# xxlong0/ESTDepth

Measured on AMD Instinct MI355X. Metric: depth frames/sec (seq_len=5, 480x640, D=64), higher is better.
Workload: dtype f32; 1 GPU; cfg2: seq_len=5, 480x640, ndepths=64, ResNet-50, Joint mode steady state (carried memory, EST on); launch=hipGraph replay, pipeline=False, graph_memory=zero-copy, conv3d_arith=f32, conv2d_arith=f32, conv3d_algo_32to32=wino3, full=False, parallelism=1 sequence per GPU

## Files before the change

estdepth_amd/csrc/conv3d_wino3.hip:

```cpp
#include <hip/hip_runtime.h>
#include <stdint.h>
#include <stdlib.h>
#include <type_traits>

#include "estd_hip.h"
#include "estd_common.h"

#ifndef ESTD_W3BD
#define ESTD_W3BD 4
#endif
#ifndef ESTD_W3_SCHED
#define ESTD_W3_SCHED 1
#endif
#ifndef ESTD_W3_WRING
#define ESTD_W3_WRING 0
#endif
#ifndef ESTD_W3_RBQ
#define ESTD_W3_RBQ 5
#endif
#ifndef ESTD_W3_TANH_HALVES
#define ESTD_W3_TANH_HALVES 1
#endif
#ifndef ESTD_W3_PFQ
#define ESTD_W3_PFQ 4
#endif
#ifndef ESTD_W3_PFQ_RB
#define ESTD_W3_PFQ_RB 8
#endif
#ifndef ESTD_W3PRIO
#define ESTD_W3PRIO 0
#endif
#ifndef ESTD_W3PK
#define ESTD_W3PK 0
#endif
#ifndef ESTD_W3_SCHED_VALU
#define ESTD_W3_SCHED_VALU 8
#endif
#ifndef ESTD_W3ABL
#define ESTD_W3ABL 0
#endif

namespace {

typedef float f32x4 __attribute__((ext_vector_type(4)));
typedef float f32x2 __attribute__((ext_vector_type(2)));
typedef unsigned int u32x4 __attribute__((__vector_size__(16)));

constexpr int TH = 8, TW = 16;
constexpr int IN_H = TH + 2, IN_W = TW + 2;
constexpr int SL_VOX = IN_H * IN_W;
constexpr int SL_CHUNKS = SL_VOX * 8;
constexpr int LINE_BYTES = IN_W * 128 + 16;
constexpr int ROW_BYTES = 4 * LINE_BYTES;
constexpr int SLICE_BYTES = LINE_BYTES;
constexpr int SLICES_BYTES = IN_H * ROW_BYTES;
constexpr int NTHREADS = 512, SIT = 3;
constexpr int RED_BYTES = 512;
constexpr int SS_BYTES = 3 * 32 * 4;
constexpr int VTAB_BYTES = SIT * NTHREADS * 4;
constexpr int XCH_BYTES = 8 * 4 * 64 * 16;
constexpr int NTAPS = 64, TAP_BYTES = 4096;
constexpr int DUMMY_BYTES = 96 * 16 + 2 * LINE_BYTES;
constexpr int XSL_BYTES = 4 * SL_VOX * 4;
constexpr int XW_BYTES = 2 * 4 * 2 * 64 * 16;
constexpr int LDS_BASE_BYTES = SLICES_BYTES + RED_BYTES + SS_BYTES + VTAB_BYTES + XCH_BYTES + DUMMY_BYTES;
#ifndef ESTD_W3_WLDS
#define ESTD_W3_WLDS 1
#endif
#ifndef ESTD_W3_WLQ0_PLAIN
#define ESTD_W3_WLQ0_PLAIN 4
#endif
constexpr int WL_N = 3;
constexpr int WL_BYTES = 2 * WL_N * 4096;
constexpr int LDS_BYTES_EXTRA = LDS_BASE_BYTES + XSL_BYTES + XW_BYTES, LDS_BYTES_PLAIN = LDS_BASE_BYTES + (ESTD_W3_WLDS ? WL_BYTES : 0);
static_assert(LDS_BYTES_EXTRA <= 160 * 1024 && LDS_BYTES_PLAIN <= 160 * 1024, "LDS budget");
constexpr unsigned OOB_OFFSET = 0xFFFFFF00u;

__device__ __forceinline__ float4 as_float4(u32x4 v)
{
    float4 f;
    __builtin_memcpy(&f, &v, 16);
    return f;
}
__device__ __forceinline__ __amdgpu_buffer_rsrc_t make_rsrc(const float* base, size_t elems)
{
    return __builtin_amdgcn_make_buffer_rsrc(const_cast<float*>(base), 0, (int)(elems * 4), 0x00020000);
}
template <int CTRL>
__device__ __forceinline__ double dpp_add_f64(double v)
{
    const unsigned long long b = __builtin_bit_cast(unsigned long long, v);
    const unsigned lo = (unsigned)__builtin_amdgcn_update_dpp(0, (int)(unsigned)b, CTRL, 0xf, 0xf, false);
    const unsigned hi = (unsigned)__builtin_amdgcn_update_dpp(0, (int)(unsigned)(b >> 32), CTRL, 0xf, 0xf, false);
    return v + __builtin_bit_cast(double, ((unsigned long long)hi << 32) | lo);
}
__device__ __forceinline__ double row16_sum_f64(double v)
{
    v = dpp_add_f64<0xB1>(v);
    v = dpp_add_f64<0x4E>(v);
    v = dpp_add_f64<0x124>(v);
    v = dpp_add_f64<0x128>(v);
    return v;
}
__device__ __forceinline__ void lds_barrier() { asm volatile("s_waitcnt lgkmcnt(0)\n\ts_barrier" ::: "memory"); }
__device__ __forceinline__ int lds_colkey_off(int col, int c) { return col * 128 + ((c ^ ((col >> 1) & 7)) << 4); }
__device__ __forceinline__ float tanh_fast(float x)
{
    const float t = __builtin_amdgcn_exp2f(x * 2.8853900817779268f);
    return 1.0f - 2.0f * __builtin_amdgcn_rcpf(t + 1.0f);
}
__device__ __forceinline__ float act_apply(float v, int act)
{
    if (act == ESTD_ACT_RELU) return v > 0.0f ? v : 0.0f;
    if (act == ESTD_ACT_TANH) return tanh_fast(v);
    return v;
}
__device__ __forceinline__ float4 f4_sub(float4 a, float4 b) { return make_float4(a.x - b.x, a.y - b.y, a.z - b.z, a.w - b.w); }
__device__ __forceinline__ float4 f4_add(float4 a, float4 b) { return make_float4(a.x + b.x, a.y + b.y, a.z + b.z, a.w + b.w); }

#ifndef ESTD_W3DEFER
#define ESTD_W3DEFER 1
#endif
template <int RBK, bool STATS, bool EXTRA>
__global__ __launch_bounds__(NTHREADS, 1) void conv3d_wino3_kernel(const estd_conv3d_desc p, int tiles_w, int tiles_h, int dpairs, int total_tiles)
{
    constexpr bool RB_ACC = RBK == 1 || RBK == 3, RB_RES = RBK == 2 || RBK == 3;
    constexpr bool DEFER = ESTD_W3DEFER != 0;
    extern __shared__ __attribute__((aligned(16))) char smem[];
    const int tid = threadIdx.x;
    const int lane = tid & 63;
    const int wave = __builtin_amdgcn_readfirstlane(tid >> 6);
    const int rq = wave & 1;
    const int nh = (wave >> 1) & 1;
    const int shh = wave >> 2;
    const int g = lane >> 4;
    const int i = lane & 15;
    const int rpl = (i >= 4 && i < 12) ? 1 : 0;
    const int cb = i < 4 ? i : i < 12 ? i - 4 : i - 8;
    const int D = p.D, H = p.H, W = p.W;
    const int HW = H * W;
    const size_t vol = (size_t)D * HW;

    int u, u_end;
    {
        const int G = gridDim.x, bid = blockIdx.x;
        const int r = ((G & 7) == 0) ? (bid & 7) * (G >> 3) + (bid >> 3) : bid;
        u = (int)((long long)total_tiles * r / G);
        u_end = (int)((long long)total_tiles * (r + 1) / G);
    }
    if (u >= u_end) return;

    float* lds_ss = reinterpret_cast<float*>(smem + SLICES_BYTES + RED_BYTES);
    if (tid < 64) lds_ss[tid] = tid < 32 ? p.scale[tid & 31] : p.shift[tid & 31];
    if (tid >= 64 && tid < 96) lds_ss[tid] = ((tid - 64) < p.act_split ? p.act_a : p.act_b) == ESTD_ACT_RELU ? 0.0f : ESTD_NO_FLOOR;
    const bool any_tanh = p.act_a == ESTD_ACT_TANH || p.act_b == ESTD_ACT_TANH;
    const bool tanh_halves = ESTD_W3_TANH_HALVES && any_tanh && (p.act_split & 15) == 0;
    const int wave_act = __builtin_amdgcn_readfirstlane(16 * nh < p.act_split ? p.act_a : p.act_b);
    unsigned* lds_vt = reinterpret_cast<unsigned*>(smem + SLICES_BYTES + RED_BYTES + SS_BYTES);
    float4* lds_xch = reinterpret_cast<float4*>(smem + SLICES_BYTES + RED_BYTES + SS_BYTES + VTAB_BYTES);
    const __amdgpu_buffer_rsrc_t rs_null = __builtin_amdgcn_make_buffer_rsrc(const_cast<float*>(p.w_wino2), 0, 0, 0x00020000);
    float* lds_x = reinterpret_cast<float*>(smem + SLICES_BYTES + RED_BYTES + SS_BYTES + VTAB_BYTES + XCH_BYTES + DUMMY_BYTES);
    char* lds_wx = smem + SLICES_BYTES + RED_BYTES + SS_BYTES + VTAB_BYTES + XCH_BYTES + DUMMY_BYTES + XSL_BYTES;
    if (EXTRA) {
        for (int e = tid; e < XW_BYTES / 16; e += NTHREADS) reinterpret_cast<float4*>(lds_wx)[e] = reinterpret_cast<const float4*>(p.w_extra)[e];
    }
    constexpr bool WL = ESTD_W3_WLDS != 0 && !EXTRA;
    constexpr int WL_Q0 = RBK == 0 ? ESTD_W3_WLQ0_PLAIN : 4;
    char* lds_wl = smem + LDS_BASE_BYTES;
    if (WL) {
        for (int e = tid; e < WL_BYTES / 16; e += NTHREADS) {
            const int blk = e >> 8, q_ = WL_Q0 + blk % WL_N, sh_ = 2 * (blk / WL_N) + (q_ & 1);
            const int src = ((((q_ >> 3) * 4 + sh_) * 2 + ((q_ >> 2) & 1)) * 2 + ((q_ >> 1) & 1));
            reinterpret_cast<float4*>(lds_wl)[e] = reinterpret_cast<const float4*>(p.w_wino2)[src * 256 + (e & 255)];
        }
    }
    const int xbase = ((4 * rq + 2 * rpl) * IN_W + 2 * cb) * 4 + g * (SL_VOX * 4);

    const __amdgpu_buffer_rsrc_t rs_w = make_rsrc(p.w_wino2, (size_t)NTAPS * 1024);
    const int wlane = lane * 16 + nh * 2048;
    int cbase[4][2][2];
#pragma unroll
    for (int j = 0; j < 4; ++j)
#pragma unroll
        for (int cc = 0; cc < 2; ++cc)
#pragma unroll
            for (int hh = 0; hh < 2; ++hh) cbase[j][cc][hh] = (4 * rq + 2 * rpl) * ROW_BYTES + lds_colkey_off(2 * cb + j, g + 4 * cc) + 8 * (hh ^ (g & 1));

    constexpr int BD = ESTD_W3BD;
    static_assert(32 % BD == 0, "the weight ring runs on across tiles");
    if (ESTD_W3PRIO == 1 && shh != 0) __builtin_amdgcn_s_setprio(1);
    while (u < u_end) {
        const int col = u / dpairs;
        int dp = u - col * dpairs;
        const int twi = col % tiles_w, c2 = col / tiles_w;
        const int thi = c2 % tiles_h, n = c2 / tiles_h;
        const int tw0 = twi * TW, th0 = thi * TH;
        const int seg_end = min(u_end, (col + 1) * dpairs);

        const __amdgpu_buffer_rsrc_t rs_in = make_rsrc(p.in_main + (size_t)n * vol * p.in_stride, vol * p.in_stride);
        __amdgpu_buffer_rsrc_t rs_res = rs_in, rs_res2 = rs_in;
        const __amdgpu_buffer_rsrc_t rs_out = make_rsrc(p.out_main + (size_t)n * vol * p.out_stride, vol * p.out_stride);
        rs_res = (RB_RES && p.residual) ? make_rsrc(p.residual + (size_t)n * vol * p.out_stride, vol * p.out_stride) : rs_null;
        rs_res2 = (RB_RES && p.residual2) ? make_rsrc(p.residual2 + (size_t)n * vol * p.out_stride, vol * p.out_stride) : rs_null;
        const __amdgpu_buffer_rsrc_t rs_ex = EXTRA ? make_rsrc(p.in_extra + (size_t)n * vol, vol) : rs_null;
        unsigned xoff = OOB_OFFSET;
        if (EXTRA && tid < SL_VOX) {
            const int zy = tid / IN_W, zx = tid % IN_W;
            const int gy = th0 - 1 + zy, gx = tw0 - 1 + zx;
            if ((unsigned)gy < (unsigned)H && (unsigned)gx < (unsigned)W) xoff = (unsigned)(gy * W + gx) * 4u;
        }
        auto load_x = [&](int pd) {
            return (unsigned)pd < (unsigned)D ? __builtin_bit_cast(float, __builtin_amdgcn_raw_buffer_load_b32(rs_ex, xoff, pd * HW * 4, 0)) : 0.0f;
        };
        const int in_slice_bytes = HW * p.in_stride * 4;
        const int out_plane_bytes = HW * p.out_stride * 4;

#pragma unroll
        for (int it = 0; it < SIT; ++it) {
            const int e = tid + it * NTHREADS;
            const int vs = e >> 3, c = e & 7;
            const int zy = vs / IN_W, zx = vs % IN_W;
            const int gy = th0 - 1 + zy, gx = tw0 - 1 + zx;
            const bool ok = e < SL_CHUNKS && (unsigned)gy < (unsigned)H && (unsigned)gx < (unsigned)W;
            lds_vt[it * NTHREADS + tid] = ok ? (unsigned)((gy * W + gx) * p.in_stride + c * 4) * 4u : OOB_OFFSET;
        }
        auto chunk_voff = [&](int it) {
            const int l = __builtin_amdgcn_mbcnt_hi(~0u, __builtin_amdgcn_mbcnt_lo(~0u, 0u));
            return lds_vt[it * NTHREADS + wave * 64 + l];
        };
        int loffk[SIT];
#pragma unroll
        for (int it = 0; it < SIT; ++it) {
            const int vs = (tid >> 3) + it * (NTHREADS / 8);
            loffk[it] = (vs / IN_W) * ROW_BYTES + lds_colkey_off(vs % IN_W, tid & 7);
        }
        const bool last_ok = tid + (SIT - 1) * NTHREADS < SL_CHUNKS;
        int loffw[SIT];
#pragma unroll
        for (int it = 0; it < SIT; ++it) loffw[it] = (it < SIT - 1 || last_ok) ? loffk[it] : (SLICES_BYTES + RED_BYTES + SS_BYTES + VTAB_BYTES + XCH_BYTES + (tid - 416) * 16);
        auto load_plane = [&](int pd, float4 (&dst)[SIT]) {
            const bool pv = (unsigned)pd < (unsigned)D;
#pragma unroll
            for (int it = 0; it < SIT; ++it)
                dst[it] = pv ? as_float4(__builtin_amdgcn_raw_buffer_load_b128(rs_in, chunk_voff(it), pd * in_slice_bytes, 0)) : make_float4(0.f, 0.f, 0.f, 0.f);
        };
        unsigned eoff[2][2];
#pragma unroll
        for (int m = 0; m < 2; ++m)
#pragma unroll
            for (int c = 0; c < 2; ++c) {
                const int y = th0 + 4 * rq + 2 * rpl + m, x = tw0 + 2 * cb + c;
                eoff[m][c] = (y < H && x < W) ? (unsigned)((y * W + x) * p.out_stride + 16 * nh + 4 * g) * 4u : OOB_OFFSET;
            }
        auto bn_act = [&](const f32x4& a, int chb, float4& v) {
            const float4 sc4 = *reinterpret_cast<const float4*>(lds_ss + chb), sh4 = *reinterpret_cast<const float4*>(lds_ss + 32 + chb);
            if (!any_tanh) {
                const float4 lo = *reinterpret_cast<const float4*>(lds_ss + 64 + chb);
                v.x = fmaxf(a[0] * sc4.x + sh4.x, lo.x);
                v.y = fmaxf(a[1] * sc4.y + sh4.y, lo.y);
                v.z = fmaxf(a[2] * sc4.z + sh4.z, lo.z);
                v.w = fmaxf(a[3] * sc4.w + sh4.w, lo.w);
                return;
            }
            if (tanh_halves) {
                const float u0 = a[0] * sc4.x + sh4.x, u1 = a[1] * sc4.y + sh4.y, u2 = a[2] * sc4.z + sh4.z, u3 = a[3] * sc4.w + sh4.w;
                if (wave_act == ESTD_ACT_TANH) { v.x = tanh_fast(u0); v.y = tanh_fast(u1); v.z = tanh_fast(u2); v.w = tanh_fast(u3); }
                else if (wave_act == ESTD_ACT_RELU) { v.x = fmaxf(u0, 0.f); v.y = fmaxf(u1, 0.f); v.z = fmaxf(u2, 0.f); v.w = fmaxf(u3, 0.f); }
                else { v.x = u0; v.y = u1; v.z = u2; v.w = u3; }
                return;
            }
            v.x = act_apply(a[0] * sc4.x + sh4.x, chb + 0 < p.act_split ? p.act_a : p.act_b);
            v.y = act_apply(a[1] * sc4.y + sh4.y, chb + 1 < p.act_split ? p.act_a : p.act_b);
            v.z = act_apply(a[2] * sc4.z + sh4.z, chb + 2 < p.act_split ? p.act_a : p.act_b);
            v.w = act_apply(a[3] * sc4.w + sh4.w, chb + 3 < p.act_split ? p.act_a : p.act_b);
        };
        struct EpiLoads { float4 r1[2], r2[2], ro[2]; };
        auto epi_issue = [&](int m, int so, const __amdgpu_buffer_rsrc_t& q1, const __amdgpu_buffer_rsrc_t& q2, const __amdgpu_buffer_rsrc_t& qo, EpiLoads& L) {
#pragma unroll
            for (int c = 0; c < 2; ++c) {
                if (RB_RES) L.r1[c] = as_float4(__builtin_amdgcn_raw_buffer_load_b128(q1, eoff[m][c], so, 0));
                if (RB_RES) L.r2[c] = as_float4(__builtin_amdgcn_raw_buffer_load_b128(q2, eoff[m][c], so, 0));
                if (RB_ACC) L.ro[c] = as_float4(__builtin_amdgcn_raw_buffer_load_b128(qo, eoff[m][c], so, 0));
            }
        };
        auto epi_finish = [&](const f32x4 (&a)[2], int m, int so, const __amdgpu_buffer_rsrc_t& qo, const EpiLoads& L) {
#pragma unroll
            for (int c = 0; c < 2; ++c) {
                float4 v;
                bn_act(a[c], 16 * nh + 4 * g, v);
                if (RB_RES) {
                    v = f4_add(f4_add(v, L.r1[c]), L.r2[c]);
                    v = make_float4(v.x * p.out_scale, v.y * p.out_scale, v.z * p.out_scale, v.w * p.out_scale);
                }
                if (RB_ACC) v = f4_add(v, L.ro[c]);
                u32x4 bits;
                __builtin_memcpy(&bits, &v, 16);
                if (!(ESTD_W3ABL & 1)) __builtin_amdgcn_raw_buffer_store_b128(bits, qo, eoff[m][c], so, 0);
            }
        };
        auto epi_plane = [&](const f32x4 (&a)[2][2], int dd) {
            const int so = dd * out_plane_bytes;
            EpiLoads L0, L1;
            epi_issue(0, so, rs_res, rs_res2, rs_out, L0);
            epi_issue(1, so, rs_res, rs_res2, rs_out, L1);
            epi_finish(a[0], 0, so, rs_out, L0);
            epi_finish(a[1], 1, so, rs_out, L1);
        };
        f32x4 py[2][2];
        int pso = 0;
        bool have_prev = false;
#pragma unroll
        for (int m = 0; m < 2; ++m)
#pragma unroll
            for (int c = 0; c < 2; ++c) py[m][c] = (f32x4){0.f, 0.f, 0.f, 0.f};

        float4 xa[SIT], xb[SIT], xc[SIT], xd[SIT];
        {
            const int d0 = 2 * dp;
            load_plane(d0 - 1, xa);
            load_plane(d0, xb);
            load_plane(d0 + 1, xc);
            load_plane(d0 + 2, xd);
        }
        float ea = 0.f, eb = 0.f, ec = 0.f, ed = 0.f;
        if (EXTRA) {
            const int d0 = 2 * dp;
            ea = load_x(d0 - 1); eb = load_x(d0); ec = load_x(d0 + 1); ed = load_x(d0 + 2);
        }
        char* xw_ptr = tid < SL_VOX ? reinterpret_cast<char*>(lds_x) + tid * 4 : smem + SLICES_BYTES + RED_BYTES + SS_BYTES + VTAB_BYTES + XCH_BYTES + (tid & 63) * 4;
        auto write_x_slice = [&](int sl) {
            if (EXTRA) *reinterpret_cast<float*>(xw_ptr + sl * (SL_VOX * 4)) = sl == 0 ? ea - ec : sl == 1 ? eb + ec : sl == 2 ? ec - eb : eb - ed;
        };
        auto write_slice = [&](int sl) {
#pragma unroll
            for (int it = 0; it < SIT; ++it) {
                if ((it < SIT - 1 || last_ok) && !(ESTD_W3ABL & 2)) {
                    const float4 v = sl == 0 ? f4_sub(xa[it], xc[it]) : sl == 1 ? f4_add(xb[it], xc[it])
                                   : sl == 2 ? f4_sub(xc[it], xb[it]) : f4_sub(xb[it], xd[it]);
                    *reinterpret_cast<float4*>(smem + loffk[it] + sl * SLICE_BYTES) = v;
                }
            }
        };
        auto shift_planes = [&]() {
#pragma unroll
            for (int it = 0; it < SIT; ++it) { xa[it] = xc[it]; xb[it] = xd[it]; }
            if (EXTRA) { ea = ec; eb = ed; }
        };
        bool first = true;
        int stats_parity = 0;
        float4 bq[BD][2];
        bool w_primed = false;

        for (; u < seg_end; ++u, ++dp) {
            const int d0 = 2 * dp;
            if (first) {
                lds_barrier();
#pragma unroll
                for (int sl = 0; sl < 4; ++sl) write_slice(sl);
#pragma unroll
                for (int sl = 0; sl < 4; ++sl) write_x_slice(sl);
                shift_planes();
                lds_barrier();
                first = false;
            }
            const bool has_next = (u + 1 < seg_end);
            const int nd = d0 + 3;
            const __amdgpu_buffer_rsrc_t rs_pf0 = (has_next && nd < D) ? rs_in : rs_null, rs_pf1 = (has_next && nd + 1 < D) ? rs_in : rs_null;
            const __amdgpu_buffer_rsrc_t rs_px0 = (EXTRA && has_next && nd < D) ? rs_ex : rs_null, rs_px1 = (EXTRA && has_next && nd + 1 < D) ? rs_ex : rs_null;

            f32x4 P[2][2][2];
            const __amdgpu_buffer_rsrc_t rp_out = have_prev ? rs_out : rs_null, rp_res = have_prev ? rs_res : rs_null, rp_res2 = have_prev ? rs_res2 : rs_null;

            auto tap_loop = [&](auto shh_c) {
                constexpr int SHH = decltype(shh_c)::value;
                constexpr int NQ = 32;
                constexpr int RA0 = SHH == 0 ? 0 : 2, RSH = SHH == 0 ? 2 : 1, RA1 = SHH == 0 ? 1 : 3;
                f32x4 m[2][4];
                f32x2 RA[4], RBs[4];
                f32x2 T[4];

                auto load_w = [&](int q, float4 (&b)[2]) {
                    const int sd = q >> 3, cc = (q >> 2) & 1, hh = (q >> 1) & 1, sh = 2 * SHH + (q & 1);
#pragma unroll
                    for (int sp = 0; sp < 2; ++sp) {
                        if (WL && q >= WL_Q0 && q < WL_Q0 + WL_N) b[sp] = *reinterpret_cast<const float4*>(lds_wl + (SHH * WL_N + q - WL_Q0) * 4096 + sp * 1024 + wlane);
                        else b[sp] = as_float4(__builtin_amdgcn_raw_buffer_load_b128(rs_w, wlane, ((((sd * 4 + sh) * 2 + cc) * 2 + hh) * TAP_BYTES) + sp * 1024, 0));
                    }
                };
                auto load_rowA = [&](int q) {
                    const int sd = q >> 3, cc = (q >> 2) & 1, hh = (q >> 1) & 1, r = (q & 1) ? RA1 : RA0;
#pragma unroll
                    for (int j = 0; j < 4; ++j) RA[j] = *reinterpret_cast<const f32x2*>(smem + cbase[j][cc][hh] + sd * SLICE_BYTES + r * ROW_BYTES);
                };
                auto load_rowB = [&](int q) {
                    const int sd = q >> 3, cc = (q >> 2) & 1, hh = (q >> 1) & 1;
#pragma unroll
                    for (int j = 0; j < 4; ++j) RBs[j] = *reinterpret_cast<const f32x2*>(smem + cbase[j][cc][hh] + sd * SLICE_BYTES + RSH * ROW_BYTES);
                };
                auto xform = [&](int q, f32x2 (&o)[4]) {
                    f32x2 X[4];
                    if (ESTD_W3PK && !(ESTD_W3ABL & 128)) {
                        auto pk_sub = [](f32x2 a, f32x2 b) { f32x2 r; asm("v_pk_add_f32 %0, %1, %2 neg_lo:[0,1] neg_hi:[0,1]" : "=v"(r) : "v"(a), "v"(b)); return r; };
                        auto pk_add = [](f32x2 a, f32x2 b) { f32x2 r; asm("v_pk_add_f32 %0, %1, %2" : "=v"(r) : "v"(a), "v"(b)); return r; };
#pragma unroll
                        for (int j = 0; j < 4; ++j) X[j] = (q & 1) == 0 ? pk_sub(RA[j], RBs[j]) : SHH == 0 ? pk_add(RA[j], RBs[j]) : pk_sub(RBs[j], RA[j]);
                        o[0] = pk_sub(X[0], X[2]); o[1] = pk_add(X[1], X[2]); o[2] = pk_sub(X[2], X[1]); o[3] = pk_sub(X[1], X[3]);
                        return;
                    }
#pragma unroll
                    for (int j = 0; j < 4; ++j) {
                        if (ESTD_W3ABL & 128) X[j] = RA[j];
                        else if ((q & 1) == 0) X[j] = RA[j] - RBs[j];
                        else X[j] = SHH == 0 ? RA[j] + RBs[j] : RBs[j] - RA[j];
                    }
                    if (ESTD_W3ABL & 128) { o[0] = X[0]; o[1] = X[1]; o[2] = X[2]; o[3] = X[3]; }
                    else { o[0] = X[0] - X[2]; o[1] = X[1] + X[2]; o[2] = X[2] - X[1]; o[3] = X[1] - X[3]; }
                };

                if (!ESTD_W3_WRING || !w_primed) {
#pragma unroll
                    for (int b = 0; b < BD - 1; ++b) load_w(b, bq[b]);
                    w_primed = true;
                }
                load_rowA(0);
                load_rowB(0);
                xform(0, T);
                load_rowA(1);
                if (EXTRA && !(ESTD_W3ABL & 256)) {
                    f32x2 xpt[3][2];
#pragma unroll
                    for (int r3 = 0; r3 < 3; ++r3)
#pragma unroll
                        for (int jp = 0; jp < 2; ++jp) {
                            const int row = r3 == 0 ? RA0 : r3 == 1 ? RSH : RA1;
                            xpt[r3][jp] = *reinterpret_cast<const f32x2*>(reinterpret_cast<const char*>(lds_x) + xbase + row * (IN_W * 4) + jp * 8);
                        }
                    float tx[2][4];
#pragma unroll
                    for (int s2 = 0; s2 < 2; ++s2) {
                        const f32x2 a0 = s2 == 0 ? xpt[0][0] : xpt[2][0], a1 = s2 == 0 ? xpt[0][1] : xpt[2][1];
                        const f32x2 X01 = s2 == 0 ? a0 - xpt[1][0] : (SHH == 0 ? a0 + xpt[1][0] : xpt[1][0] - a0);
                        const f32x2 X23 = s2 == 0 ? a1 - xpt[1][1] : (SHH == 0 ? a1 + xpt[1][1] : xpt[1][1] - a1);
                        tx[s2][0] = X01.x - X23.x; tx[s2][1] = X01.y + X23.x; tx[s2][2] = X23.x - X01.y; tx[s2][3] = X01.y - X23.y;
                    }
#pragma unroll
                    for (int pl_ = 0; pl_ < 2; ++pl_) {
                        f32x4 mx[2][4];
#pragma unroll
                        for (int s2 = 0; s2 < 2; ++s2) {
                            const float4 w4 = *reinterpret_cast<const float4*>(lds_wx + ((pl_ * 4 + 2 * SHH + s2) * 2 + nh) * 1024 + lane * 16);
                            mx[s2][0] = __builtin_amdgcn_mfma_f32_16x16x4f32(w4.x, tx[s2][0], (f32x4){0.f, 0.f, 0.f, 0.f}, 0, 0, 0);
                            mx[s2][1] = __builtin_amdgcn_mfma_f32_16x16x4f32(w4.y, tx[s2][1], (f32x4){0.f, 0.f, 0.f, 0.f}, 0, 0, 0);
                            mx[s2][2] = __builtin_amdgcn_mfma_f32_16x16x4f32(w4.z, tx[s2][2], (f32x4){0.f, 0.f, 0.f, 0.f}, 0, 0, 0);
                            mx[s2][3] = __builtin_amdgcn_mfma_f32_16x16x4f32(w4.w, tx[s2][3], (f32x4){0.f, 0.f, 0.f, 0.f}, 0, 0, 0);
                        }
#pragma unroll
                        for (int c = 0; c < 2; ++c) {
                            const f32x4 v0_ = c == 0 ? mx[0][0] + mx[0][1] + mx[0][2] : mx[0][1] - mx[0][2] - mx[0][3];
                            const f32x4 v1_ = c == 0 ? mx[1][0] + mx[1][1] + mx[1][2] : mx[1][1] - mx[1][2] - mx[1][3];
                            if (SHH == 0) { P[pl_][0][c] = v0_ + v1_; P[pl_][1][c] = v1_; }
                            else          { P[pl_][0][c] = v0_;       P[pl_][1][c] = -(v0_ + v1_); }
                        }
                    }
                } else if (EXTRA) {
#pragma unroll
                    for (int pl_ = 0; pl_ < 2; ++pl_)
#pragma unroll
                        for (int r = 0; r < 2; ++r)
#pragma unroll
                            for (int c = 0; c < 2; ++c) P[pl_][r][c] = (f32x4){0.f, 0.f, 0.f, 0.f};
                }
                unsigned vo_next = 0;
                EpiLoads pl, pl1;
                constexpr int PF_Q = RBK != 0 ? ESTD_W3_PFQ_RB : ESTD_W3_PFQ;
                constexpr int RW_Q = 22;
                __builtin_amdgcn_sched_barrier(0);

#pragma clang loop unroll(full)
                for (int q = 0; q < NQ; ++q) {
                    const int sd = q >> 3, sl = q & 1;
                    if (q == RW_Q) lds_barrier();
                    if (q >= RW_Q && q < RW_Q + 9 && !(ESTD_W3ABL & 2)) {
                        const int sl_w = (q - RW_Q) / SIT, it = (q - RW_Q) % SIT;
                        const float4 v = sl_w == 0 ? f4_sub(xa[it], xc[it]) : sl_w == 1 ? f4_add(xb[it], xc[it]) : f4_sub(xc[it], xb[it]);
                        *reinterpret_cast<float4*>(smem + loffw[it] + sl_w * SLICE_BYTES) = v;
                    }
                    if ((ESTD_W3_WRING || q + BD - 1 < NQ) && !(ESTD_W3ABL & 8)) load_w((q + BD - 1) % NQ, bq[(q + BD - 1) % BD]);
                    if (q >= PF_Q && q < PF_Q + 12 && ((q - PF_Q) & 1) == 0 && !(ESTD_W3ABL & 16)) {
                        const int idx = (q - PF_Q) >> 1, it = idx % SIT;
                        if (idx < SIT) xc[it] = as_float4(__builtin_amdgcn_raw_buffer_load_b128(rs_pf0, vo_next, nd * in_slice_bytes, 0));
                        else           xd[it] = as_float4(__builtin_amdgcn_raw_buffer_load_b128(rs_pf1, vo_next, (nd + 1) * in_slice_bytes, 0));
                    }
                    if (EXTRA) {
                        if (q == 16) ec = __builtin_bit_cast(float, __builtin_amdgcn_raw_buffer_load_b32(rs_px0, xoff, nd * HW * 4, 0));
                        if (q == 17) ed = __builtin_bit_cast(float, __builtin_amdgcn_raw_buffer_load_b32(rs_px1, xoff, (nd + 1) * HW * 4, 0));
                        if (q >= RW_Q && q < RW_Q + 4) write_x_slice(q - RW_Q);
                    }
                    if (DEFER) {
                        constexpr bool RB = RBK != 0;
                        constexpr int RBQ = ESTD_W3_RBQ;
                        if (RB && q == 0) epi_issue(0, pso, rp_res, rp_res2, rp_out, pl);
                        if (RB && q == 1) epi_issue(1, pso, rp_res, rp_res2, rp_out, pl1);
                        if (q == (RB ? RBQ : 1)) epi_finish(py[0], 0, pso, rp_out, pl);
                        if (q == (RB ? RBQ + 1 : 2)) epi_finish(py[1], 1, pso, rp_out, pl1);
                    }
                    if (ESTD_W3_SCHED == 0) __builtin_amdgcn_sched_barrier(0);
                    const int cur = (ESTD_W3ABL & 8) ? 0 : q % BD;
                    f32x2 Tn[4];
#pragma unroll
                    for (int e = 0; e < 2; ++e)
#pragma unroll
                        for (int sw = 0; sw < 4; ++sw) {
                            const float4 b4 = bq[cur][sw >> 1];
                            const float b = (sw & 1) == 0 ? (e == 0 ? b4.x : b4.y) : (e == 0 ? b4.z : b4.w);
                            const bool first_product = (q & 7) < 2 && e == 0;
                            const f32x4 c_in = first_product ? (f32x4){0.f, 0.f, 0.f, 0.f} : m[sl][sw];
                            m[sl][sw] = __builtin_amdgcn_mfma_f32_16x16x4f32(b, T[sw][e], c_in, 0, 0, 0);
                        }
                    if (q + 1 < NQ) xform(q + 1, Tn);
                    if (q + 2 < NQ) {
                        load_rowA(q + 2);
                        if (((q + 2) & 1) == 0) load_rowB(q + 2);
                    }
                    if (q + 1 >= PF_Q && q + 1 < PF_Q + 12 && ((q + 1 - PF_Q) & 1) == 0 && !(ESTD_W3ABL & 16)) vo_next = chunk_voff(((q + 1 - PF_Q) >> 1) % SIT);
                    if (ESTD_W3_SCHED == 0) {
                        __builtin_amdgcn_sched_group_barrier(0x008, 4, 0);
                        __builtin_amdgcn_sched_group_barrier(0x002, 4, 0);
                        __builtin_amdgcn_sched_group_barrier(0x008, 4, 0);
                        __builtin_amdgcn_sched_group_barrier(0x002, 4, 0);
                        __builtin_amdgcn_sched_group_barrier(0x100, 8, 0);
                    } else {
#pragma unroll
                        for (int gq = 0; gq < 4; ++gq) {
                            if (EXTRA && (q & 7) == 4) __builtin_amdgcn_sched_group_barrier(0x008, 4, 0);
                            else __builtin_amdgcn_sched_group_barrier(0x008, 2, 0);
                            __builtin_amdgcn_sched_group_barrier(0x020, 1, 0);
                            __builtin_amdgcn_sched_group_barrier(0x002, ESTD_W3_SCHED_VALU, 0);
                            __builtin_amdgcn_sched_group_barrier(0x100, 2, 0);
                            __builtin_amdgcn_sched_group_barrier(0x200, 1, 0);
                        }
                    }
                    if (q + 1 < NQ) {
#pragma unroll
                        for (int sw = 0; sw < 4; ++sw) T[sw] = Tn[sw];
                    }
                    __builtin_amdgcn_sched_barrier(0);
                    if ((q & 7) == 7 && !(ESTD_W3ABL & 32)) {
                        f32x4 z[2][2];
#pragma unroll
                        for (int c = 0; c < 2; ++c) {
                            const f32x4 v0_ = c == 0 ? m[0][0] + m[0][1] + m[0][2] : m[0][1] - m[0][2] - m[0][3];
                            const f32x4 v1_ = c == 0 ? m[1][0] + m[1][1] + m[1][2] : m[1][1] - m[1][2] - m[1][3];
                            if (SHH == 0) { z[0][c] = v0_ + v1_; z[1][c] = v1_; }
                            else          { z[0][c] = v0_;       z[1][c] = -(v0_ + v1_); }
                        }
#pragma unroll
                        for (int r = 0; r < 2; ++r)
#pragma unroll
                            for (int c = 0; c < 2; ++c) {
                                if (sd == 0) { if (EXTRA) P[0][r][c] += z[r][c]; else P[0][r][c] = z[r][c]; }
                                else if (sd == 1) { P[0][r][c] += z[r][c]; if (EXTRA) P[1][r][c] += z[r][c]; else P[1][r][c] = z[r][c]; }
                                else if (sd == 2) { P[0][r][c] += z[r][c]; P[1][r][c] -= z[r][c]; }
                                else P[1][r][c] -= z[r][c];
                            }
                        __builtin_amdgcn_sched_barrier(0);
                    }
                }
                if (ESTD_W3ABL & 32) {
#pragma unroll
                    for (int r = 0; r < 2; ++r)
#pragma unroll
                        for (int c = 0; c < 2; ++c) { P[0][r][c] = m[0][2 * r + c]; P[1][r][c] = m[1][2 * r + c]; }
                }
                float4* xw = lds_xch + (wave * 4) * 64 + lane;
#pragma unroll
                for (int r = 0; r < 2; ++r)
#pragma unroll
                    for (int c = 0; c < 2; ++c) {
                        const f32x4 snd = P[1 - SHH][r][c];
                        xw[(2 * r + c) * 64] = make_float4(snd[0], snd[1], snd[2], snd[3]);
                    }
                lds_barrier();
                const float4* xr = lds_xch + ((wave ^ 4) * 4) * 64 + lane;
#pragma unroll
                for (int r = 0; r < 2; ++r)
#pragma unroll
                    for (int c = 0; c < 2; ++c) {
                        const float4 o = xr[(2 * r + c) * 64];
                        P[0][r][c] = P[SHH][r][c] + (f32x4){o.x, o.y, o.z, o.w};
                    }
            };
            if (shh == 0) tap_loop(std::integral_constant<int, 0>{});
            else tap_loop(std::integral_constant<int, 1>{});

            if (STATS) {
                double* red = reinterpret_cast<double*>(smem + SLICES_BYTES) + (stats_parity ? 32 : 0);
                stats_parity ^= 1;
                double v0_ = 0.0, v1_ = 0.0;
                const int chb = 16 * nh + 4 * g;
                const float4 sc4 = *reinterpret_cast<const float4*>(lds_ss + chb), sh4 = *reinterpret_cast<const float4*>(lds_ss + 32 + chb);
                const float scv[4] = {sc4.x, sc4.y, sc4.z, sc4.w}, shv[4] = {sh4.x, sh4.y, sh4.z, sh4.w};
#pragma unroll
                for (int m = 0; m < 2; ++m)
#pragma unroll
                    for (int c = 0; c < 2; ++c)
                        if (eoff[m][c] != OOB_OFFSET) {
#pragma unroll
                            for (int r = 0; r < 4; ++r) { const double uu = (double)(P[0][m][c][r] * scv[r] + shv[r]); v0_ += uu; v1_ += uu * uu; }
                        }
                v0_ = row16_sum_f64(v0_); v1_ = row16_sum_f64(v1_);
#pragma unroll
                for (int o = 16; o <= 32; o <<= 1) { v0_ += __shfl_xor(v0_, o); v1_ += __shfl_xor(v1_, o); }
                if (lane == 0) { red[((shh * 2 + nh) * 2 + rq) * 2] = v0_; red[((shh * 2 + nh) * 2 + rq) * 2 + 1] = v1_; }
                __syncthreads();
                if (tid < 8) {
                    const int pl_ = tid >> 2, grp = (tid >> 1) & 1, qq = tid & 1;
                    if (d0 + pl_ < D) {
                        const double tot = red[((pl_ * 2 + grp) * 2 + 0) * 2 + qq] + red[((pl_ * 2 + grp) * 2 + 1) * 2 + qq];
                        const size_t tile_id = (((size_t)n * D + d0 + pl_) * tiles_h + thi) * tiles_w + twi;
                        p.stats_partials[tile_id * 4 + grp * 2 + qq] = tot;
                    }
                }
            }
            if (has_next) {
                write_slice(3);
                shift_planes();
            }
            if (DEFER && has_next) {
#pragma unroll
                for (int m = 0; m < 2; ++m)
#pragma unroll
                    for (int c = 0; c < 2; ++c) py[m][c] = P[0][m][c];
                pso = (d0 + shh) * out_plane_bytes;
                have_prev = true;
            } else {
                if (d0 + shh < D) epi_plane(P[0], d0 + shh);
                have_prev = false;
            }
        }
    }
}

constexpr int PERSISTENT_WGS = 256;

}

extern "C" int estd_conv3d_k3_wino3(const estd_conv3d_desc* dp, estd_stream_t s)
{
    if (!dp) return ESTD_ERR_ARG;
    const estd_conv3d_desc& d = *dp;
    if (d.N <= 0 || d.D <= 0 || d.H <= 0 || d.W <= 0) return ESTD_ERR_ARG;
    if (!d.in_main || !d.w_wino2 || !d.scale || !d.shift || !d.out_main) return ESTD_ERR_ARG;
    if (d.cin_main != 32 || d.n_tiles != 2 || d.out_head || d.out_extra || d.gate_r) return ESTD_ERR_UNSUPPORTED;
    const bool extra = d.in_extra != nullptr;
    if (extra != (d.w_extra != nullptr)) return ESTD_ERR_ARG;
    if (d.in_stride < 32 || (d.in_stride & 3) || d.out_stride < 32 || (d.out_stride & 3) || ((d.act_split & 1) && d.act_split < 32)) return ESTD_ERR_ARG;
    const int tiles_w = (d.W + TW - 1) / TW, tiles_h = (d.H + TH - 1) / TH, dpairs = (d.D + 1) / 2;
    const long long total = (long long)d.N * dpairs * tiles_h * tiles_w;
    if (total > 0x7fffffffLL) return ESTD_ERR_ARG;
    {
        const long long vox = (long long)d.D * d.H * d.W;
        const int widest = d.in_stride > d.out_stride ? d.in_stride : d.out_stride;
        if (vox * widest * 4 >= 0x7fffff00LL) return ESTD_ERR_UNSUPPORTED;
    }
    const int slots = estd_persistent_wgs(PERSISTENT_WGS / 256);
    int grid = total < slots ? (int)total : slots;
    if (grid >= 8) grid &= ~7;
    const bool res_any = d.residual || d.residual2 || d.out_scale != 1.0f;
    const int rbk = (!res_any && !d.accumulate) ? 0 : (!res_any ? 1 : (!d.accumulate ? 2 : 3));
    if (d.stats_partials && rbk != 0) return ESTD_ERR_UNSUPPORTED;
#define ESTD_W3_LAUNCH(RBV, STV, EXV)                                                                                                           \
    do {                                                                                                                             \
        estd_allow_dynamic_lds<conv3d_wino3_kernel<RBV, STV, EXV>>(EXV ? LDS_BYTES_EXTRA : LDS_BYTES_PLAIN);                                                                 \
        hipLaunchKernelGGL((conv3d_wino3_kernel<RBV, STV, EXV>), dim3(grid), dim3(NTHREADS), EXV ? LDS_BYTES_EXTRA : LDS_BYTES_PLAIN, estd_stream(s), d, tiles_w, tiles_h,   \
                           dpairs, (int)total);                                                                                      \
    } while (0)
    if (extra && (rbk != 0 || d.stats_partials)) return ESTD_ERR_UNSUPPORTED;
    switch (rbk) {
    case 0: if (extra) ESTD_W3_LAUNCH(0, false, true); else if (d.stats_partials) ESTD_W3_LAUNCH(0, true, false); else ESTD_W3_LAUNCH(0, false, false); break;
    case 1: ESTD_W3_LAUNCH(1, false, false); break;
    case 2: ESTD_W3_LAUNCH(2, false, false); break;
    default: ESTD_W3_LAUNCH(3, false, false); break;
    }
#undef ESTD_W3_LAUNCH
    return ESTD_LAUNCH_CHECK();
}
```

Baseline: 199.4 depth frames/s.

## Split Winograd conv3d tap loop across four spatial-shift wave pairs

Adds a SPLIT mode (on by default for non-stats, non-extra variants) where each wave pair handles one of four spatial shifts for all 32 output channels, instead of the old split of two shifts by two channel halves. Each wave now owns one output row, and partial sums are combined through a larger LDS exchange area with a barrier. Fewer weights are staged in LDS, and a new epilogue timing knob is added. A small s_nop is also inserted after each buffer store. The aim is to rebalance MFMA work and improve input-row reuse per wave, at the cost of extra LDS exchange traffic and more complex reduction.

```diff
diff --git a/estdepth_amd/csrc/conv3d_wino3.hip b/estdepth_amd/csrc/conv3d_wino3.hip
--- a/estdepth_amd/csrc/conv3d_wino3.hip
+++ b/estdepth_amd/csrc/conv3d_wino3.hip
@@ -18,6 +18,9 @@
 #ifndef ESTD_W3_RBQ
 #define ESTD_W3_RBQ 5
 #endif
+#ifndef ESTD_W3_RBQ_SPLIT
+#define ESTD_W3_RBQ_SPLIT 7
+#endif
 #ifndef ESTD_W3_TANH_HALVES
 #define ESTD_W3_TANH_HALVES 1
 #endif
@@ -35,6 +38,9 @@
 #endif
 #ifndef ESTD_W3_SCHED_VALU
 #define ESTD_W3_SCHED_VALU 8
+#endif
+#ifndef ESTD_W3_SPLIT
+#define ESTD_W3_SPLIT 1
 #endif
 #ifndef ESTD_W3ABL
 #define ESTD_W3ABL 0
@@ -58,22 +64,25 @@
 constexpr int RED_BYTES = 512;
 constexpr int SS_BYTES = 3 * 32 * 4;
 constexpr int VTAB_BYTES = SIT * NTHREADS * 4;
-constexpr int XCH_BYTES = 8 * 4 * 64 * 16;
+constexpr int XCH_SLOT = 4 * 64 * 16;
+constexpr int xch_bytes(bool split) { return (split ? 12 : 8) * XCH_SLOT; }
 constexpr int NTAPS = 64, TAP_BYTES = 4096;
 constexpr int DUMMY_BYTES = 96 * 16 + 2 * LINE_BYTES;
 constexpr int XSL_BYTES = 4 * SL_VOX * 4;
 constexpr int XW_BYTES = 2 * 4 * 2 * 64 * 16;
-constexpr int LDS_BASE_BYTES = SLICES_BYTES + RED_BYTES + SS_BYTES + VTAB_BYTES + XCH_BYTES + DUMMY_BYTES;
+constexpr int lds_base_bytes(bool split) { return SLICES_BYTES + RED_BYTES + SS_BYTES + VTAB_BYTES + xch_bytes(split) + DUMMY_BYTES; }
 #ifndef ESTD_W3_WLDS
 #define ESTD_W3_WLDS 1
 #endif
 #ifndef ESTD_W3_WLQ0_PLAIN
 #define ESTD_W3_WLQ0_PLAIN 4
 #endif
-constexpr int WL_N = 3;
-constexpr int WL_BYTES = 2 * WL_N * 4096;
-constexpr int LDS_BYTES_EXTRA = LDS_BASE_BYTES + XSL_BYTES + XW_BYTES, LDS_BYTES_PLAIN = LDS_BASE_BYTES + (ESTD_W3_WLDS ? WL_BYTES : 0);
-static_assert(LDS_BYTES_EXTRA <= 160 * 1024 && LDS_BYTES_PLAIN <= 160 * 1024, "LDS budget");
+constexpr int wl_n(bool split) { return split ? 1 : 3; }
+constexpr int wl_bytes(bool split) { return split ? 4 * wl_n(true) * 2048 : 2 * wl_n(false) * 4096; }
+constexpr int lds_bytes(bool split, bool extra) { return lds_base_bytes(split) + (extra ? XSL_BYTES + XW_BYTES : ESTD_W3_WLDS ? wl_bytes(split) : 0); }
+static_assert(lds_bytes(false, true) <= 160 * 1024 && lds_bytes(false, false) <= 160 * 1024 && lds_bytes(true, false) <= 160 * 1024, "LDS budget");
+template <int RBK, bool STATS, bool EXTRA>
+constexpr bool w3_split() { return ESTD_W3_SPLIT != 0 && !STATS && !EXTRA; }
 constexpr unsigned OOB_OFFSET = 0xFFFFFF00u;
 
 __device__ __forceinline__ float4 as_float4(u32x4 v)
@@ -126,13 +135,16 @@
 {
     constexpr bool RB_ACC = RBK == 1 || RBK == 3, RB_RES = RBK == 2 || RBK == 3;
     constexpr bool DEFER = ESTD_W3DEFER != 0;
+    constexpr bool SPLIT = w3_split<RBK, STATS, EXTRA>();
+    constexpr int XCH_BYTES = xch_bytes(SPLIT), LDS_BASE_BYTES = lds_base_bytes(SPLIT), WL_N = wl_n(SPLIT), WL_BYTES = wl_bytes(SPLIT);
     extern __shared__ __attribute__((aligned(16))) char smem[];
     const int tid = threadIdx.x;
     const int lane = tid & 63;
     const int wave = __builtin_amdgcn_readfirstlane(tid >> 6);
     const int rq = wave & 1;
-    const int nh = (wave >> 1) & 1;
-    const int shh = wave >> 2;
+    const int nh = SPLIT ? 0 : (wave >> 1) & 1;
+    const int shh = SPLIT ? (wave >> 1) & 1 : wave >> 2;
+    const int yr = wave >> 2;
     const int g = lane >> 4;
     const int i = lane & 15;
     const int rpl = (i >= 4 && i < 12) ? 1 : 0;
@@ -156,6 +168,7 @@
     const bool any_tanh = p.act_a == ESTD_ACT_TANH || p.act_b == ESTD_ACT_TANH;
     const bool tanh_halves = ESTD_W3_TANH_HALVES && any_tanh && (p.act_split & 15) == 0;
     const int wave_act = __builtin_amdgcn_readfirstlane(16 * nh < p.act_split ? p.act_a : p.act_b);
+    const int wave_act_hi = __builtin_amdgcn_readfirstlane(16 < p.act_split ? p.act_a : p.act_b);
     unsigned* lds_vt = reinterpret_cast<unsigned*>(smem + SLICES_BYTES + RED_BYTES + SS_BYTES);
     float4* lds_xch = reinterpret_cast<float4*>(smem + SLICES_BYTES + RED_BYTES + SS_BYTES + VTAB_BYTES);
     const __amdgpu_buffer_rsrc_t rs_null = __builtin_amdgcn_make_buffer_rsrc(const_cast<float*>(p.w_wino2), 0, 0, 0x00020000);
@@ -169,6 +182,12 @@
     char* lds_wl = smem + LDS_BASE_BYTES;
     if (WL) {
         for (int e = tid; e < WL_BYTES / 16; e += NTHREADS) {
+            if (SPLIT) {
+                const int blk = e >> 7, q_ = WL_Q0 + blk % WL_N, sh_ = blk / WL_N;
+                const int src = ((((q_ >> 3) * 4 + sh_) * 2 + ((q_ >> 2) & 1)) * 2 + ((q_ >> 1) & 1));
+                reinterpret_cast<float4*>(lds_wl)[e] = reinterpret_cast<const float4*>(p.w_wino2)[src * 256 + (q_ & 1) * 128 + (e & 127)];
+                continue;
+            }
             const int blk = e >> 8, q_ = WL_Q0 + blk % WL_N, sh_ = 2 * (blk / WL_N) + (q_ & 1);
             const int src = ((((q_ >> 3) * 4 + sh_) * 2 + ((q_ >> 2) & 1)) * 2 + ((q_ >> 1) & 1));
             reinterpret_cast<float4*>(lds_wl)[e] = reinterpret_cast<const float4*>(p.w_wino2)[src * 256 + (e & 255)];
@@ -249,10 +268,10 @@
         for (int m = 0; m < 2; ++m)
 #pragma unroll
             for (int c = 0; c < 2; ++c) {
-                const int y = th0 + 4 * rq + 2 * rpl + m, x = tw0 + 2 * cb + c;
-                eoff[m][c] = (y < H && x < W) ? (unsigned)((y * W + x) * p.out_stride + 16 * nh + 4 * g) * 4u : OOB_OFFSET;
-            }
-        auto bn_act = [&](const f32x4& a, int chb, float4& v) {
+                const int y = th0 + 4 * rq + 2 * rpl + (SPLIT ? yr : m), x = tw0 + 2 * cb + c;
+                eoff[m][c] = (y < H && x < W) ? (unsigned)((y * W + x) * p.out_stride + 16 * (SPLIT ? m : nh) + 4 * g) * 4u : OOB_OFFSET;
+            }
+        auto bn_act = [&](const f32x4& a, int chb, float4& v, int half) {
             const float4 sc4 = *reinterpret_cast<const float4*>(lds_ss + chb), sh4 = *reinterpret_cast<const float4*>(lds_ss + 32 + chb);
             if (!any_tanh) {
                 const float4 lo = *reinterpret_cast<const float4*>(lds_ss + 64 + chb);
@@ -264,8 +283,9 @@
             }
             if (tanh_halves) {
                 const float u0 = a[0] * sc4.x + sh4.x, u1 = a[1] * sc4.y + sh4.y, u2 = a[2] * sc4.z + sh4.z, u3 = a[3] * sc4.w + sh4.w;
-                if (wave_act == ESTD_ACT_TANH) { v.x = tanh_fast(u0); v.y = tanh_fast(u1); v.z = tanh_fast(u2); v.w = tanh_fast(u3); }
-                else if (wave_act == ESTD_ACT_RELU) { v.x = fmaxf(u0, 0.f); v.y = fmaxf(u1, 0.f); v.z = fmaxf(u2, 0.f); v.w = fmaxf(u3, 0.f); }
+                const int wact = (SPLIT && half) ? wave_act_hi : wave_act;
+                if (wact == ESTD_ACT_TANH) { v.x = tanh_fast(u0); v.y = tanh_fast(u1); v.z = tanh_fast(u2); v.w = tanh_fast(u3); }
+                else if (wact == ESTD_ACT_RELU) { v.x = fmaxf(u0, 0.f); v.y = fmaxf(u1, 0.f); v.z = fmaxf(u2, 0.f); v.w = fmaxf(u3, 0.f); }
                 else { v.x = u0; v.y = u1; v.z = u2; v.w = u3; }
                 return;
             }
@@ -287,7 +307,7 @@
 #pragma unroll
             for (int c = 0; c < 2; ++c) {
                 float4 v;
-                bn_act(a[c], 16 * nh + 4 * g, v);
+                bn_act(a[c], 16 * (SPLIT ? m : nh) + 4 * g, v, m);
                 if (RB_RES) {
                     v = f4_add(f4_add(v, L.r1[c]), L.r2[c]);
                     v = make_float4(v.x * p.out_scale, v.y * p.out_scale, v.z * p.out_scale, v.w * p.out_scale);
@@ -295,7 +315,10 @@
                 if (RB_ACC) v = f4_add(v, L.ro[c]);
                 u32x4 bits;
                 __builtin_memcpy(&bits, &v, 16);
-                if (!(ESTD_W3ABL & 1)) __builtin_amdgcn_raw_buffer_store_b128(bits, qo, eoff[m][c], so, 0);
+                if (!(ESTD_W3ABL & 1)) {
+                    __builtin_amdgcn_raw_buffer_store_b128(bits, qo, eoff[m][c], so, 0);
+                    asm volatile("s_nop 3" ::"v"(bits));
+                }
             }
         };
         auto epi_plane = [&](const f32x4 (&a)[2][2], int dd) {
@@ -590,8 +613,155 @@
                         P[0][r][c] = P[SHH][r][c] + (f32x4){o.x, o.y, o.z, o.w};
                     }
             };
-            if (shh == 0) tap_loop(std::integral_constant<int, 0>{});
-            else tap_loop(std::integral_constant<int, 1>{});
+
+            auto tap_loop_split = [&](auto sh_c) {
+                constexpr int SH = decltype(sh_c)::value;
+                constexpr int NQ = 32;
+                constexpr int RA_ = SH == 0 ? 0 : SH == 2 ? 2 : 1, RB_ = SH == 0 ? 2 : SH == 1 ? 2 : SH == 2 ? 1 : 3;
+                f32x4 m[2][4];
+                f32x2 RA[4], RBs[4];
+                f32x2 T[4];
+
+                auto load_w = [&](int q, float4 (&b)[2]) {
+                    const int sd = q >> 3, cc = (q >> 2) & 1, hh = (q >> 1) & 1, half = q & 1;
+#pragma unroll
+                    for (int sp = 0; sp < 2; ++sp) {
+                        if (WL && q >= WL_Q0 && q < WL_Q0 + WL_N) b[sp] = *reinterpret_cast<const float4*>(lds_wl + (SH * WL_N + q - WL_Q0) * 2048 + sp * 1024 + wlane);
+                        else b[sp] = as_float4(__builtin_amdgcn_raw_buffer_load_b128(rs_w, wlane, ((((sd * 4 + SH) * 2 + cc) * 2 + hh) * TAP_BYTES) + half * 2048 + sp * 1024, 0));
+                    }
+                };
+                auto load_rows = [&](int un) {
+                    const int sd = un >> 2, cc = (un >> 1) & 1, hh = un & 1;
+#pragma unroll
+                    for (int j = 0; j < 4; ++j) RA[j] = *reinterpret_cast<const f32x2*>(smem + cbase[j][cc][hh] + sd * SLICE_BYTES + RA_ * ROW_BYTES);
+#pragma unroll
+                    for (int j = 0; j < 4; ++j) RBs[j] = *reinterpret_cast<const f32x2*>(smem + cbase[j][cc][hh] + sd * SLICE_BYTES + RB_ * ROW_BYTES);
+                };
+                auto xform = [&](f32x2 (&o)[4]) {
+                    f32x2 X[4];
+#pragma unroll
+                    for (int j = 0; j < 4; ++j) X[j] = (ESTD_W3ABL & 128) ? RA[j] : SH == 1 ? RA[j] + RBs[j] : RA[j] - RBs[j];
+                    if (ESTD_W3ABL & 128) { o[0] = X[0]; o[1] = X[1]; o[2] = X[2]; o[3] = X[3]; }
+                    else { o[0] = X[0] - X[2]; o[1] = X[1] + X[2]; o[2] = X[2] - X[1]; o[3] = X[1] - X[3]; }
+                };
+#pragma unroll
+                for (int b = 0; b < BD - 1; ++b) load_w(b, bq[b]);
+                load_rows(0);
+                xform(T);
+                unsigned vo_next = 0;
+                EpiLoads pl, pl1;
+                constexpr int PF_Q = RBK != 0 ? ESTD_W3_PFQ_RB : ESTD_W3_PFQ;
+                constexpr int RW_Q = 22;
+                __builtin_amdgcn_sched_barrier(0);
+
+#pragma clang loop unroll(full)
+                for (int q = 0; q < NQ; ++q) {
+                    const int sd = q >> 3, half = q & 1;
+                    if (q == RW_Q) lds_barrier();
+                    if (q >= RW_Q && q < RW_Q + 9 && !(ESTD_W3ABL & 2)) {
+                        const int sl_w = (q - RW_Q) / SIT, it = (q - RW_Q) % SIT;
+                        const float4 v = sl_w == 0 ? f4_sub(xa[it], xc[it]) : sl_w == 1 ? f4_add(xb[it], xc[it]) : f4_sub(xc[it], xb[it]);
+                        *reinterpret_cast<float4*>(smem + loffw[it] + sl_w * SLICE_BYTES) = v;
+                    }
+                    if (q + BD - 1 < NQ && !(ESTD_W3ABL & 8)) load_w(q + BD - 1, bq[(q + BD - 1) % BD]);
+                    if (q >= PF_Q && q < PF_Q + 12 && ((q - PF_Q) & 1) == 0 && !(ESTD_W3ABL & 16)) {
+                        const int idx = (q - PF_Q) >> 1, it = idx % SIT;
+                        if (idx < SIT) xc[it] = as_float4(__builtin_amdgcn_raw_buffer_load_b128(rs_pf0, vo_next, nd * in_slice_bytes, 0));
+                        else           xd[it] = as_float4(__builtin_amdgcn_raw_buffer_load_b128(rs_pf1, vo_next, (nd + 1) * in_slice_bytes, 0));
+                    }
+                    if (DEFER) {
+                        constexpr bool RB = RBK != 0;
+                        constexpr int RBQ = ESTD_W3_RBQ_SPLIT;
+                        if (RB && q == 0) epi_issue(0, pso, rp_res, rp_res2, rp_out, pl);
+                        if (RB && q == 1) epi_issue(1, pso, rp_res, rp_res2, rp_out, pl1);
+                        if (q == (RB ? RBQ : 1)) epi_finish(py[0], 0, pso, rp_out, pl);
+                        if (q == (RB ? RBQ + 1 : 2)) epi_finish(py[1], 1, pso, rp_out, pl1);
+                    }
+                    const int cur = (ESTD_W3ABL & 8) ? 0 : q % BD;
+                    f32x2 Tn[4];
+                    if (half == 0 && q + 2 < NQ) load_rows((q >> 1) + 1);
+#pragma unroll
+                    for (int e = 0; e < 2; ++e)
+#pragma unroll
+                        for (int sw = 0; sw < 4; ++sw) {
+                            const float4 b4 = bq[cur][sw >> 1];
+                            const float b = (sw & 1) == 0 ? (e == 0 ? b4.x : b4.y) : (e == 0 ? b4.z : b4.w);
+                            const bool first_product = (q & 7) < 2 && e == 0;
+                            const f32x4 c_in = first_product ? (f32x4){0.f, 0.f, 0.f, 0.f} : m[half][sw];
+                            m[half][sw] = __builtin_amdgcn_mfma_f32_16x16x4f32(b, T[sw][e], c_in, 0, 0, 0);
+                        }
+                    if (half == 1 && q + 1 < NQ) xform(Tn);
+                    if (q + 1 >= PF_Q && q + 1 < PF_Q + 12 && ((q + 1 - PF_Q) & 1) == 0 && !(ESTD_W3ABL & 16)) vo_next = chunk_voff(((q + 1 - PF_Q) >> 1) % SIT);
+#pragma unroll
+                    for (int gq = 0; gq < 4; ++gq) {
+                        __builtin_amdgcn_sched_group_barrier(0x008, 2, 0);
+                        __builtin_amdgcn_sched_group_barrier(0x020, 1, 0);
+                        __builtin_amdgcn_sched_group_barrier(0x002, ESTD_W3_SCHED_VALU, 0);
+                        __builtin_amdgcn_sched_group_barrier(0x100, 2, 0);
+                        __builtin_amdgcn_sched_group_barrier(0x200, 1, 0);
+                    }
+                    if (half == 1 && q + 1 < NQ) {
+#pragma unroll
+                        for (int sw = 0; sw < 4; ++sw) T[sw] = Tn[sw];
+                    }
+                    __builtin_amdgcn_sched_barrier(0);
+                    if ((q & 7) == 7 && !(ESTD_W3ABL & 32)) {
+#pragma unroll
+                        for (int h = 0; h < 2; ++h)
+#pragma unroll
+                            for (int c = 0; c < 2; ++c) {
+                                const f32x4 z = c == 0 ? m[h][0] + m[h][1] + m[h][2] : m[h][1] - m[h][2] - m[h][3];
+                                if (sd == 0) P[0][h][c] = z;
+                                else if (sd == 1) { P[0][h][c] += z; P[1][h][c] = z; }
+                                else if (sd == 2) { P[0][h][c] += z; P[1][h][c] -= z; }
+                                else P[1][h][c] -= z;
+                            }
+                        __builtin_amdgcn_sched_barrier(0);
+                    }
+                }
+                if (ESTD_W3ABL & 32) {
+#pragma unroll
+                    for (int h = 0; h < 2; ++h)
+#pragma unroll
+                        for (int c = 0; c < 2; ++c) { P[0][h][c] = m[h][c]; P[1][h][c] = m[h][2 + c]; }
+                }
+                float4* xs = lds_xch + rq * 6 * 256 + lane;
+                auto put = [&](int slot, const f32x4 (&a)[2][2]) {
+#pragma unroll
+                    for (int h = 0; h < 2; ++h)
+#pragma unroll
+                        for (int c = 0; c < 2; ++c) xs[slot * 256 + (2 * h + c) * 64] = make_float4(a[h][c][0], a[h][c][1], a[h][c][2], a[h][c][3]);
+                };
+                auto get = [&](int slot, int h, int c) {
+                    const float4 o = xs[slot * 256 + (2 * h + c) * 64];
+                    return (f32x4){o.x, o.y, o.z, o.w};
+                };
+                if (SH == 0) put(0, P[1]);
+                if (SH == 1) { put(1, P[0]); put(2, P[1]); }
+                if (SH == 2) { put(3, P[0]); put(4, P[1]); }
+                if (SH == 3) put(5, P[0]);
+                lds_barrier();
+#pragma unroll
+                for (int h = 0; h < 2; ++h)
+#pragma unroll
+                    for (int c = 0; c < 2; ++c) {
+                        if (SH == 0) P[0][h][c] = P[0][h][c] + get(1, h, c) + get(3, h, c);
+                        if (SH == 1) P[0][h][c] = P[1][h][c] + get(0, h, c) + get(4, h, c);
+                        if (SH == 2) P[0][h][c] = get(1, h, c) - P[0][h][c] - get(5, h, c);
+                        if (SH == 3) P[0][h][c] = get(2, h, c) - get(4, h, c) - P[1][h][c];
+                    }
+            };
+            if constexpr (SPLIT) {
+                switch (wave >> 1) {
+                case 0: tap_loop_split(std::integral_constant<int, 0>{}); break;
+                case 1: tap_loop_split(std::integral_constant<int, 1>{}); break;
+                case 2: tap_loop_split(std::integral_constant<int, 2>{}); break;
+                default: tap_loop_split(std::integral_constant<int, 3>{}); break;
+                }
+            } else {
+                if (shh == 0) tap_loop(std::integral_constant<int, 0>{});
+                else tap_loop(std::integral_constant<int, 1>{});
+            }
 
             if (STATS) {
                 double* red = reinterpret_cast<double*>(smem + SLICES_BYTES) + (stats_parity ? 32 : 0);
@@ -671,8 +841,9 @@
     if (d.stats_partials && rbk != 0) return ESTD_ERR_UNSUPPORTED;
 #define ESTD_W3_LAUNCH(RBV, STV, EXV)                                                                                                           \
     do {                                                                                                                             \
-        estd_allow_dynamic_lds<conv3d_wino3_kernel<RBV, STV, EXV>>(EXV ? LDS_BYTES_EXTRA : LDS_BYTES_PLAIN);                                                                 \
-        hipLaunchKernelGGL((conv3d_wino3_kernel<RBV, STV, EXV>), dim3(grid), dim3(NTHREADS), EXV ? LDS_BYTES_EXTRA : LDS_BYTES_PLAIN, estd_stream(s), d, tiles_w, tiles_h,   \
+        constexpr int lds_ = lds_bytes(w3_split<RBV, STV, EXV>(), EXV);                                                              \
+        estd_allow_dynamic_lds<conv3d_wino3_kernel<RBV, STV, EXV>>(lds_);                                                            \
+        hipLaunchKernelGGL((conv3d_wino3_kernel<RBV, STV, EXV>), dim3(grid), dim3(NTHREADS), lds_, estd_stream(s), d, tiles_w, tiles_h,   \
                            dpairs, (int)total);                                                                                      \
     } while (0)
     if (extra && (rbk != 0 || d.stats_partials)) return ESTD_ERR_UNSUPPORTED;
```

Result: faster. 201.7 depth frames/s, median of 6 (+1.2%).
